# Irish-77/adapting-2D-ViTs-for-3D-point-cloud-understanding

Measured on NVIDIA B200. Metric: tokenized clouds/sec (FPS+kNN+embed), higher is better.
Workload: dtype bf16

## Files before the change

### adapting-2d-vits-for-3d-point-cloud-understanding_b200/csrc/embed_fused.cu

```cuda
#include <vector>

#include "tc_common.cuh"

namespace p3tok {

constexpr int FU_CH_WARPS = 8, FU_OUT_WARPS = 8;
constexpr int FU_THREADS = (3 + FU_CH_WARPS + FU_OUT_WARPS) * 32;
constexpr int FU_CHUNK = 128;
constexpr int FU_CH_BYTES = 2 * 16384;
constexpr int FU_RA_BOX = 64 * 128;
constexpr int FU_MAX_RA = 32, FU_MAX_RB = 16;
constexpr int FU_SMEM = 227 * 1024;
constexpr int FU_L1_WSTRIDE = 76;
constexpr int FU_L1_STAGE = 128 * 16 + 4 * 16;
constexpr int FU_L1_BYTES = 2 * FU_L1_STAGE;

struct FusedParams {
  int M, K0, N1, N2;
  int num_pairs;
  int ra_slots, rb_slots, rb_box;
  int nch;
  int nacc;
  int nq, nq_rows;
  int xtile;
  int a_reuse;
  const float* bias_a;
  const float* gbias;
  int rows_per_group;
  const float* bias_b;
  int store_out;
  float* out_max;
  __nv_bfloat16* out_max_bf16;
  int max_relu;
  unsigned long long* trace;
  const float4* l1_rel;
  const float4* l1_ctr;
  const float* l1_w;
  int l1_relu;
};
__device__ __forceinline__ void fu_trace(const FusedParams& p, int it, int j, int slot, long long v) {
  if (p.trace && blockIdx.x == 0 && it < 4 && j < 16) p.trace[((size_t)it * 16 + j) * 16 + slot] = (unsigned long long)v;
}

__global__ void __launch_bounds__(FU_THREADS, 1)
tc_fused_kernel(const __grid_constant__ CUtensorMap tmA, const __grid_constant__ CUtensorMap tmWa,
                const __grid_constant__ CUtensorMap tmWb, const __grid_constant__ CUtensorMap tmC, const FusedParams p) {
  extern __shared__ uint8_t smem_raw[];
  uint8_t* smem = reinterpret_cast<uint8_t*>((reinterpret_cast<uintptr_t>(smem_raw) + 1023) & ~(uintptr_t)1023);
  const int KB0 = p.K0 / 64, NC = p.N1 / FU_CHUNK, NQ = p.nq;
  uint8_t* sA0 = smem;
  uint8_t* sCH = sA0 + KB0 * 16384;
  uint8_t* sRA = sCH + p.nch * FU_CH_BYTES;
  uint8_t* sRB = sRA + p.ra_slots * FU_RA_BOX;
  uint8_t* sST = sRB + p.rb_slots * p.rb_box;
  float* sba = reinterpret_cast<float*>(sST + (p.store_out ? FU_OUT_WARPS * 4096 : 0));
  float* sbb = sba + p.N1;
  float* sgb = sbb + p.N2;
  const bool L1 = p.l1_rel != nullptr;
  uint8_t* sl1 = reinterpret_cast<uint8_t*>((reinterpret_cast<uintptr_t>(sgb + FU_CH_WARPS * 64) + 15) & ~(uintptr_t)15);
  uint64_t* bars = reinterpret_cast<uint64_t*>((reinterpret_cast<uintptr_t>(sl1 + (L1 ? 2 * FU_L1_STAGE : 0)) + 7) & ~(uintptr_t)7);
  uint64_t* a0_full = bars;
  uint64_t* a0_empty = bars + 1;
  uint64_t* acc3_full = bars + 2;
  uint64_t* acc3_empty = bars + 3;
  uint64_t* acc2_full = bars + 4;
  uint64_t* acc2_empty = bars + 6;
  uint64_t* ch_full = bars + 8;
  uint64_t* ch_empty = bars + 10;
  uint64_t* ra_full = bars + 12;
  uint64_t* ra_empty = bars + 44;
  uint64_t* rb_full = bars + 76;
  uint64_t* rb_empty = bars + 92;
  uint64_t* l1_full = bars + 108;
  uint64_t* l1_empty = bars + 110;
  uint32_t* tmem_slot = reinterpret_cast<uint32_t*>(bars + 112);

  const int warp = __shfl_sync(0xffffffffu, (int)(threadIdx.x >> 5), 0);
  const int lane = threadIdx.x & 31;
  const int rank = (int)cluster_ctarank();
  const int pair_id = blockIdx.x >> 1, pair_stride = gridDim.x >> 1;

  if (threadIdx.x == 0) {
    asm volatile("prefetch.tensormap [%0];" ::"l"(reinterpret_cast<uint64_t>(&tmA)) : "memory");
    asm volatile("prefetch.tensormap [%0];" ::"l"(reinterpret_cast<uint64_t>(&tmWa)) : "memory");
    asm volatile("prefetch.tensormap [%0];" ::"l"(reinterpret_cast<uint64_t>(&tmWb)) : "memory");
    mbar_init(a0_full, L1 ? 2 * FU_CH_WARPS : 1);
    mbar_init(a0_empty, 1);
    for (int b = 0; b < 2; ++b) { mbar_init(&l1_full[b], 1); mbar_init(&l1_empty[b], FU_CH_WARPS); }
    mbar_init(acc3_full, 1);
    mbar_init(acc3_empty, 2 * FU_OUT_WARPS);
    for (int b = 0; b < 2; ++b) {
      mbar_init(&acc2_full[b], 1);
      mbar_init(&acc2_empty[b], 2 * FU_CH_WARPS);
      mbar_init(&ch_full[b], 2 * FU_CH_WARPS);
      mbar_init(&ch_empty[b], 1);
    }
    for (int s = 0; s < FU_MAX_RA; ++s) { mbar_init(&ra_full[s], 1); mbar_init(&ra_empty[s], 1); }
    for (int s = 0; s < FU_MAX_RB; ++s) { mbar_init(&rb_full[s], 1); mbar_init(&rb_empty[s], 1); }
    asm volatile("fence.mbarrier_init.release.cluster;" ::: "memory");
  }
  for (int i = threadIdx.x; i < p.N1; i += FU_THREADS) sba[i] = p.bias_a ? p.bias_a[i] : 0.f;
  int bb_nonzero = 0;
  for (int i = threadIdx.x; i < p.N2; i += FU_THREADS) {
    const float b = p.bias_b ? p.bias_b[i] : 0.f;
    sbb[i] = b;
    bb_nonzero |= (b != 0.f);
  }
  if (warp == 1) {
    asm volatile("tcgen05.alloc.cta_group::2.sync.aligned.shared::cta.b32 [%0], %1;" ::"r"(smem_u32(tmem_slot)), "r"(512));
    asm volatile("tcgen05.relinquish_alloc_permit.cta_group::2.sync.aligned;" ::);
  }
  tc_fence_before();
  const bool has_bb = __syncthreads_or(bb_nonzero) != 0;
  cluster_sync_all();
  tc_fence_after();
  const uint32_t tmem_base = *tmem_slot;
  const int nq_rows = p.nq_rows;
  const uint32_t acc_col0 = 512u - (uint32_t)p.nacc * FU_CHUNK;

  if (warp == 0) {
    const bool issuer = elect_one();
    int rs = 0;
    uint32_t rph = 0;
    int it = 0;
    auto l1_load = [&](int t, int tp_t) {
      const int sb = t & 1;
      mbar_wait(&l1_empty[sb], ((uint32_t)(t >> 1) & 1) ^ 1);
      if (issuer) {
        const int64_t mt_t = 2 * (int64_t)tp_t + rank;
        uint8_t* dst = sl1 + sb * FU_L1_STAGE;
        mbar_expect_tx(&l1_full[sb], (uint32_t)FU_L1_STAGE);
        asm volatile("cp.async.bulk.shared::cluster.global.mbarrier::complete_tx::bytes [%0], [%1], %2, [%3];" ::"r"(smem_u32(dst)),
                     "l"(reinterpret_cast<uint64_t>(p.l1_rel + mt_t * TC_BM)), "r"(128 * 16), "r"(smem_u32(&l1_full[sb]))
                     : "memory");
        asm volatile("cp.async.bulk.shared::cluster.global.mbarrier::complete_tx::bytes [%0], [%1], %2, [%3];" ::"r"(smem_u32(dst + 128 * 16)),
                     "l"(reinterpret_cast<uint64_t>(p.l1_ctr + mt_t * (TC_BM / 32))), "r"(4 * 16), "r"(smem_u32(&l1_full[sb]))
                     : "memory");
      }
      __syncwarp();
    };
    if (L1 && pair_id < p.num_pairs) l1_load(0, pair_id);
    for (int tp = pair_id; tp < p.num_pairs; tp += pair_stride, ++it) {
      const int mt = 2 * tp + rank;
      if (L1) {
        if (tp + pair_stride < p.num_pairs) l1_load(it + 1, tp + pair_stride);
      } else {
        mbar_wait(a0_empty, (uint32_t)(it & 1) ^ 1);
        if (issuer) {
          if (rank == 0) mbar_expect_tx(a0_full, 2u * (uint32_t)KB0 * 16384u);
          for (int kb = 0; kb < KB0; ++kb) tma_load_2d_pair(sA0 + kb * 16384, &tmA, a0_full, kb * 64, mt * TC_BM);
        }
      }
      __syncwarp();
      for (int j = 0; j < NC; ++j) {
        for (int kb = 0; kb < KB0; ++kb) {
          mbar_wait(&ra_empty[rs], rph ^ 1);
          if (issuer) {
            if (rank == 0) mbar_expect_tx(&ra_full[rs], 2u * FU_RA_BOX);
            tma_load_2d_pair(sRA + rs * FU_RA_BOX, &tmWa, &ra_full[rs], kb * 64, j * FU_CHUNK + rank * (FU_CHUNK / 2));
          }
          __syncwarp();
          if (++rs == p.ra_slots) { rs = 0; rph ^= 1; }
        }
      }
    }
  } else if (warp == 2 + FU_CH_WARPS + FU_OUT_WARPS) {
    const bool issuer = elect_one();
    int rs = 0;
    uint32_t rph = 0;
    for (int tp = pair_id; tp < p.num_pairs; tp += pair_stride) {
      for (int j = 0; j < NC; ++j) {
        for (int kq = 0; kq < 2 * NQ; ++kq) {
          const int kb2 = kq / NQ, qd = kq - kb2 * NQ;
          mbar_wait(&rb_empty[rs], rph ^ 1);
          if (issuer) {
            if (rank == 0) mbar_expect_tx(&rb_full[rs], 2u * (uint32_t)p.rb_box);
            tma_load_2d_pair(sRB + rs * p.rb_box, &tmWb, &rb_full[rs], j * FU_CHUNK + kb2 * 64, qd * nq_rows + rank * (nq_rows / 2));
          }
          __syncwarp();
          if (++rs == p.rb_slots) { rs = 0; rph ^= 1; }
        }
      }
    }
  } else if (warp == 1) {
    if (rank == 0) {
      const bool issuer = elect_one();
      const uint64_t dconst = umma_desc_sw128(0);
      const uint32_t idesc_a = (1u << 4) | (1u << 7) | (1u << 10) | ((uint32_t)(FU_CHUNK >> 3) << 17) | ((uint32_t)((2 * TC_BM) >> 4) << 24);
      const uint32_t idesc_b = (1u << 4) | (1u << 7) | (1u << 10) | ((uint32_t)(nq_rows >> 3) << 17) | ((uint32_t)((2 * TC_BM) >> 4) << 24);
      const uint32_t a0_base = smem_u32(sA0) >> 4, ch_base = smem_u32(sCH) >> 4;
      const uint32_t ra_base = smem_u32(sRA) >> 4, rb_base = smem_u32(sRB) >> 4;
      int ras = 0, rbs = 0;
      uint32_t raph = 0, rbph = 0;
      uint32_t gc = 0;
      uint32_t gcb = 0;
      int it = 0;
      auto issue_A = [&](bool last_of_tile) {
        const uint32_t b = p.nacc == 2 ? (gc & 1) : 0u;
        const uint32_t use = p.nacc == 2 ? (gc >> 1) : gc;
        mbar_wait(&acc2_empty[b], (use & 1) ^ 1);
        tc_fence_after();
        const uint32_t d = tmem_base + acc_col0 + b * FU_CHUNK;
        for (int kb = 0; kb < KB0; ++kb) {
          mbar_wait(&ra_full[ras], raph);
          tc_fence_after();
          if (issuer) {
            const uint64_t ad = dconst | (uint64_t)(a0_base + kb * (16384 >> 4));
            const uint64_t bd = dconst | (uint64_t)(ra_base + ras * (FU_RA_BOX >> 4));
#pragma unroll
            for (int k = 0; k < 4; ++k) tc_mma_pair(d, ad + 2 * k, bd + 2 * k, idesc_a, (uint32_t)((kb | k) != 0));
            tc_commit_pair(&ra_empty[ras]);
          }
          __syncwarp();
          if (++ras == p.ra_slots) { ras = 0; raph ^= 1; }
        }
        if (issuer) {
          tc_commit_pair(&acc2_full[b]);
          if (last_of_tile) tc_commit_pair(a0_empty);
        }
        __syncwarp();
        ++gc;
      };
      auto first_A = [&](int tile_it) {
        if (issuer) fu_trace(p, tile_it, 0, 4, clock64());
        mbar_wait(a0_full, (uint32_t)(tile_it & 1));
        if (issuer) fu_trace(p, tile_it, 0, 5, clock64());
        tc_fence_after();
        issue_A(NC == 1);
        if (issuer) fu_trace(p, tile_it, 0, 6, clock64());
      };
      if (p.xtile && pair_id < p.num_pairs) first_A(0);
      for (int tp = pair_id; tp < p.num_pairs; tp += pair_stride, ++it) {
        if (!p.xtile) first_A(it);
        for (int j = 0; j < NC; ++j) {
          if (j + 1 < NC) issue_A(j + 1 == NC - 1);
          else if (p.xtile && tp + pair_stride < p.num_pairs) first_A(it + 1);
          const uint32_t b = p.nch == 2 ? (gcb & 1) : 0u;
          const uint32_t cuse = p.nch == 2 ? (gcb >> 1) : gcb;
          if (issuer) fu_trace(p, it, j, 0, clock64());
          mbar_wait(&ch_full[b], cuse & 1);
          if (issuer) fu_trace(p, it, j, 1, clock64());
          if (j == 0) mbar_wait(acc3_empty, (uint32_t)(it & 1) ^ 1);
          tc_fence_after();
          if (NQ == 2 && p.a_reuse) {
            for (int kb2 = 0; kb2 < 2; ++kb2) {
              const int s0 = rbs;
              const uint32_t ph0 = rbph;
              if (++rbs == p.rb_slots) { rbs = 0; rbph ^= 1; }
              const int s1 = rbs;
              const uint32_t ph1 = rbph;
              if (++rbs == p.rb_slots) { rbs = 0; rbph ^= 1; }
              mbar_wait(&rb_full[s0], ph0);
              if (issuer && kb2 == 0) fu_trace(p, it, j, 2, clock64());
              mbar_wait(&rb_full[s1], ph1);
              if (issuer && kb2 == 1) fu_trace(p, it, j, 3, clock64());
              tc_fence_after();
              if (issuer) {
                const uint64_t ad = dconst | (uint64_t)(ch_base + b * (FU_CH_BYTES >> 4) + kb2 * (16384 >> 4));
                const uint64_t bd0 = dconst | (uint64_t)(rb_base + s0 * (p.rb_box >> 4));
                const uint64_t bd1 = dconst | (uint64_t)(rb_base + s1 * (p.rb_box >> 4));
#pragma unroll
                for (int k = 0; k < 4; ++k) {
                  const uint32_t acc = (uint32_t)((j | kb2 | k) != 0);
                  tc_mma_pair_a<1>(tmem_base, ad + 2 * k, bd0 + 2 * k, idesc_b, acc);
                  tc_mma_pair_a<0>(tmem_base + (uint32_t)nq_rows, ad + 2 * k, bd1 + 2 * k, idesc_b, acc);
                }
                tc_commit_pair(&rb_empty[s0]);
                tc_commit_pair(&rb_empty[s1]);
              }
              __syncwarp();
            }
          } else
          for (int kq = 0; kq < 2 * NQ; ++kq) {
            const int kb2 = kq / NQ, qd = kq - kb2 * NQ;
            mbar_wait(&rb_full[rbs], rbph);
            if (issuer && kq == 0) fu_trace(p, it, j, 2, clock64());
            if (issuer && kq == 2 * NQ - 1) fu_trace(p, it, j, 3, clock64());
            tc_fence_after();
            if (issuer) {
              const uint64_t ad = dconst | (uint64_t)(ch_base + b * (FU_CH_BYTES >> 4) + kb2 * (16384 >> 4));
              const uint64_t bd = dconst | (uint64_t)(rb_base + rbs * (p.rb_box >> 4));
              const uint32_t d = tmem_base + (uint32_t)(qd * nq_rows);
#pragma unroll
              for (int k = 0; k < 4; ++k) tc_mma_pair(d, ad + 2 * k, bd + 2 * k, idesc_b, (uint32_t)((j | kb2 | k) != 0));
              tc_commit_pair(&rb_empty[rbs]);
            }
            __syncwarp();
            if (++rbs == p.rb_slots) { rbs = 0; rbph ^= 1; }
          }
          if (issuer) {
            fu_trace(p, it, j, 7, clock64());
            tc_commit_pair(&ch_empty[b]);
            if (j == NC - 1) tc_commit_pair(acc3_full);
          }
          __syncwarp();
          ++gcb;
        }
      }
    }
  } else if (warp < 2 + FU_CH_WARPS) {
    const int ew = warp - 2;
    const int q = warp & 3, h = ew >> 2;
    const uint32_t lane_field = (uint32_t)(q * 32) << 16;
    const int trow = q * 32 + lane;
    float* my_sgb = sgb + ew * 64;
    uint32_t gc = 0;
    int itc = 0;
    const bool tr = (warp == 2 && lane == 0);
    for (int tp = pair_id; tp < p.num_pairs; tp += pair_stride, ++itc) {
      const int row0 = (2 * tp + rank) * TC_BM + q * 32;
      const float* gb_row = (p.gbias && row0 < p.M) ? p.gbias + (size_t)(row0 / p.rows_per_group) * p.N1 : nullptr;
      for (int j = 0; j < NC; ++j, ++gc) {
        const uint32_t ba = p.nacc == 2 ? (gc & 1) : 0u, use = p.nacc == 2 ? (gc >> 1) : gc;
        const uint32_t bc = p.nch == 2 ? (gc & 1) : 0u, cuse = p.nch == 2 ? (gc >> 1) : gc;
        const int c0 = j * FU_CHUNK + h * 64;
        float2 gpre = make_float2(0.f, 0.f);
        if (gb_row) gpre = __ldg(reinterpret_cast<const float2*>(gb_row + c0) + lane);
        if (tr) fu_trace(p, itc, j, 8, clock64());
        mbar_wait(&acc2_full[ba], use & 1);
        if (tr) fu_trace(p, itc, j, 9, clock64());
        tc_fence_after();
        const uint32_t taddr = tmem_base + lane_field + acc_col0 + ba * FU_CHUNK + h * 64;
        float v[32];
        uint32_t pk[32];
        tc_ld32_issue(taddr, v);
        if (gb_row) {
          *reinterpret_cast<float2*>(my_sgb + 2 * lane) = gpre;
          __syncwarp();
        }
#pragma unroll
        for (int half = 0; half < 2; ++half) {
          tc_ld_wait();
          if (half == 1) {
            tc_fence_before();
            __syncwarp();
            if (lane == 0) mbar_arrive_cta(&acc2_empty[ba], 0);
          }
          const uint32_t sb = smem_u32(sba + c0 + 32 * half), sg = smem_u32(my_sgb + 32 * half);
// ... 59 lines not shown
        for (int c = 0; c < 4; ++c) {
#pragma unroll
          for (int j = 0; j < 8; j += 2) fma2(base[j], base[j + 1], wc[c * 8 + j], wc[c * 8 + j + 1], cv[c], cv[c], base[j], base[j + 1]);
        }
      }
      const float4* relp = reinterpret_cast<const float4*>(sl1 + sb * FU_L1_STAGE) + ew * 16;
      const uint32_t dst0 = smem_u32(sA0) + (uint32_t)(lane >> 3) * 16384u;
#pragma unroll
      for (int r4 = 0; r4 < 16; r4 += 4) {
        uint32_t pk[4][4];
#pragma unroll
        for (int rr = 0; rr < 4; ++rr) {
          const float4 xv = relp[r4 + rr];
          const float xr[4] = {xv.x, xv.y, xv.z, xv.w};
          float a[8];
#pragma unroll
          for (int j = 0; j < 8; ++j) a[j] = base[j];
#pragma unroll
          for (int c = 0; c < 4; ++c) {
#pragma unroll
            for (int j = 0; j < 8; j += 2) fma2(a[j], a[j + 1], wr[c * 8 + j], wr[c * 8 + j + 1], xr[c], xr[c], a[j], a[j + 1]);
          }
#pragma unroll
          for (int j = 0; j < 4; ++j) pk[rr][j] = p.l1_relu ? pack_bf16x2_relu(a[2 * j], a[2 * j + 1]) : pack_bf16x2(a[2 * j], a[2 * j + 1]);
        }
        if (r4 == 0) mbar_wait(a0_empty, (uint32_t)(t & 1) ^ 1);
#pragma unroll
        for (int rr = 0; rr < 4; ++rr) {
          const uint32_t trow_ = (uint32_t)(ew * 16 + r4 + rr);
          const uint32_t dst = dst0 + trow_ * 128u + ((((uint32_t)lane & 7u) ^ (trow_ & 7u)) << 4);
          asm volatile("st.shared.v4.b32 [%0], {%1, %2, %3, %4};" ::"r"(dst), "r"(pk[rr][0]), "r"(pk[rr][1]), "r"(pk[rr][2]), "r"(pk[rr][3]) : "memory");
        }
      }
      asm volatile("fence.proxy.async.shared::cta;" ::: "memory");
      __syncwarp();
      if (lane == 0) {
        mbar_arrive(&l1_empty[sb]);
        mbar_arrive_cta(a0_full, 0);
      }
    };
    if (L1 && pair_id < p.num_pairs) produce_a0(0);
    int it = 0;
    for (int tp = pair_id; tp < p.num_pairs; tp += pair_stride, ++it) {
      if (L1 && tp + pair_stride < p.num_pairs) produce_a0(it + 1);
      const int row0 = (2 * tp + rank) * TC_BM + q * 32;
      const int row = row0 + lane;
      const bool row_ok = row < p.M;
      const int nvalid = p.M - row0 >= 32 ? 32 : (p.M - row0 > 0 ? p.M - row0 : 0);
      const bool tr = (warp == 2 + FU_CH_WARPS && lane == 0);
      if (tr) fu_trace(p, it, 0, 12, clock64());
      mbar_wait(acc3_full, (uint32_t)(it & 1));
      if (tr) fu_trace(p, it, 0, 13, clock64());
      tc_fence_after();
      bool released = false;
      if (!p.store_out) {
        for (int gi = h; gi < ngroups; gi += 2) {
          const int n0 = gi * 64;
          const bool last = gi + 2 >= ngroups;
          float a0[16], b0[16], a1[16], b1[16];
          const uint32_t t0 = tmem_base + lane_field + (uint32_t)n0;
          tc_ld16x256_x4_issue(t0, a0);
          tc_ld16x256_x4_issue(t0 + (16u << 16), b0);
          tc_ld16x256_x4_issue(t0 + 32u, a1);
          tc_ld16x256_x4_issue(t0 + 32u + (16u << 16), b1);
          tc_ld_wait();
          if (last) {
            tc_fence_before();
            __syncwarp();
            if (lane == 0) mbar_arrive_cta(acc3_empty, 0);
            if (tr) fu_trace(p, it, 0, 14, clock64());
            released = true;
          }
          float m0 = rows_max_frag(a0, b0, lane, nvalid) + sbb[n0 + fcol];
          float m1 = rows_max_frag(a1, b1, lane, nvalid) + sbb[n0 + 32 + fcol];
          if (p.max_relu) { m0 = fmaxf(m0, 0.f); m1 = fmaxf(m1, 0.f); }
          if (row0 < p.M) {
            const size_t o = (size_t)(row0 >> 5) * p.N2 + n0 + fcol;
            if (p.out_max) { p.out_max[o] = m0; p.out_max[o + 32] = m1; }
            if (p.out_max_bf16) { p.out_max_bf16[o] = __float2bfloat16_rn(m0); p.out_max_bf16[o + 32] = __float2bfloat16_rn(m1); }
          }
        }
      } else {
        for (int gi = h; gi < ngroups; gi += 2) {
          const int n0 = gi * 64;
          const bool last = gi + 2 >= ngroups;
#pragma unroll
          for (int half = 0; half < 2; ++half) {
            float v[32];
            tc_ld32_issue(tmem_base + lane_field + (uint32_t)(n0 + half * 32), v);
            tc_ld_wait();
            if (last && half == 1) {
              tc_fence_before();
              __syncwarp();
              if (lane == 0) mbar_arrive_cta(acc3_empty, 0);
              if (tr) fu_trace(p, it, 0, 14, clock64());
              released = true;
            }
            if (has_bb) {
#pragma unroll
              for (int i = 0; i < 8; ++i) {
                const float4 b4 = *reinterpret_cast<const float4*>(sbb + n0 + half * 32 + 4 * i);
                v[4 * i] += b4.x; v[4 * i + 1] += b4.y; v[4 * i + 2] += b4.z; v[4 * i + 3] += b4.w;
              }
            }
            if (half == 0) {
              if (lane == 0) asm volatile("cp.async.bulk.wait_group.read 0;" ::: "memory");
              __syncwarp();
            }
            const uint32_t rbase = smem_u32(stg) + lane * 128;
#pragma unroll
            for (int pc = 0; pc < 4; ++pc) {
              const uint32_t a = rbase + (((uint32_t)(pc + 4 * half) ^ (lane & 7)) << 4);
              asm volatile("st.shared.v4.b32 [%0], {%1, %2, %3, %4};" ::"r"(a), "r"(pack_bf16x2(v[pc * 8], v[pc * 8 + 1])),
                           "r"(pack_bf16x2(v[pc * 8 + 2], v[pc * 8 + 3])), "r"(pack_bf16x2(v[pc * 8 + 4], v[pc * 8 + 5])),
                           "r"(pack_bf16x2(v[pc * 8 + 6], v[pc * 8 + 7]))
                           : "memory");
            }
            if (p.out_max) {
              if (!row_ok) {
#pragma unroll
                for (int i = 0; i < 32; ++i) v[i] = -3.0e38f;
              }
              float m = warp_rows_max(v, lane);
              if (p.max_relu) m = fmaxf(m, 0.f);
              if (row0 < p.M) p.out_max[(size_t)(row0 >> 5) * p.N2 + n0 + half * 32 + lane] = m;
            }
          }
          asm volatile("fence.proxy.async.shared::cta;" ::: "memory");
          __syncwarp();
          if (lane == 0 && row0 < p.M) {
            asm volatile("cp.async.bulk.tensor.2d.global.shared::cta.bulk_group [%0, {%2, %3}], [%1];" ::"l"(
                             reinterpret_cast<uint64_t>(&tmC)),
                         "r"(smem_u32(stg)), "r"(n0), "r"(row0)
                         : "memory");
            asm volatile("cp.async.bulk.commit_group;" ::: "memory");
          }
          if (p.out_max_bf16 && row0 < p.M) {
            uint32_t m = box_rows_max_bf16x2(smem_u32(stg), lane, nvalid);
            if (p.max_relu) asm("max.bf16x2 %0, %0, %1;" : "+r"(m) : "r"(0u));
            *reinterpret_cast<uint32_t*>(p.out_max_bf16 + (size_t)(row0 >> 5) * p.N2 + n0 + 2 * lane) = m;
          }
          __syncwarp();
        }
      }
      if (tr) fu_trace(p, it, 0, 15, clock64());
      if (!released) {
        tc_fence_before();
        __syncwarp();
        if (lane == 0) mbar_arrive_cta(acc3_empty, 0);
      }
    }
    if (lane == 0) asm volatile("cp.async.bulk.wait_group 0;" ::: "memory");
  }
  tc_fence_before();
  __syncthreads();
  cluster_sync_all();
  if (warp == 1) {
    tc_fence_after();
    asm volatile("tcgen05.dealloc.cta_group::2.sync.aligned.b32 %0, %1;" ::"r"(tmem_base), "r"(512));
  }
}

static bool fused_rings_n(int K0, int N1, int N2, bool store_out, int nch, bool l1, int& ra_slots, int& rb_slots, int& rb_box) {
  const int nq = N2 > 256 ? 2 : 1;
  rb_box = (N2 / nq / 2) * 128;
  const int fixed = (K0 / 64) * 16384 + nch * FU_CH_BYTES + (store_out ? FU_OUT_WARPS * 4096 : 0) +
                    (N1 + N2 + FU_CH_WARPS * 64) * 4 + (l1 ? FU_L1_BYTES + 16 : 0) + 116 * 8 + 64 + 1024;
  const int left = FU_SMEM - fixed;
  if (left < 2 * FU_RA_BOX + 2 * rb_box) return false;
  const int chunk_a = (K0 / 64) * FU_RA_BOX, chunk_b = 2 * nq * rb_box;
  ra_slots = (int)((int64_t)left * chunk_a / (chunk_a + chunk_b)) / FU_RA_BOX;
  if (ra_slots < 2) ra_slots = 2;
  if (ra_slots > FU_MAX_RA) ra_slots = FU_MAX_RA;
  rb_slots = (left - ra_slots * FU_RA_BOX) / rb_box;
  if (rb_slots > FU_MAX_RB) rb_slots = FU_MAX_RB;
  return rb_slots >= 2;
}

static bool fused_rings(int K0, int N1, int N2, bool store_out, bool l1, int& nch, int& ra_slots, int& rb_slots, int& rb_box) {
  nch = 2;
  if (fused_rings_n(K0, N1, N2, store_out, 2, l1, ra_slots, rb_slots, rb_box) && ra_slots >= 4 && rb_slots >= 3) return true;
  nch = 1;
  return fused_rings_n(K0, N1, N2, store_out, 1, l1, ra_slots, rb_slots, rb_box);
}

bool tc_fused_supported(int K0, int N1, int N2, int64_t rows_per_group, bool has_gbias) {
  if (K0 % 64 || N1 % FU_CHUNK || N2 % 64) return false;
  if (K0 < 64 || K0 > 384 || N2 < 64 || N2 > 384 || N1 < FU_CHUNK || N1 > 2048) return false;
  if (N2 > 256 && (N2 / 2) % 16) return false;
  if (has_gbias && (rows_per_group % 32 != 0)) return false;
  int nch, ra, rb, box;
  return fused_rings(K0, N1, N2, !has_gbias, false, nch, ra, rb, box);
}

__global__ void fused_l1_pack_kernel(const __nv_bfloat16* __restrict__ W, const float* __restrict__ bias, int C, float* __restrict__ out) {
  const int lane = blockIdx.x, i = threadIdx.x;
  float v = 0.f;
  if (i < 64) {
    const int half = i >> 5, c = (i & 31) >> 3, j = i & 7;
    if (c < C) v = __bfloat162float(W[(size_t)(8 * lane + j) * (2 * C) + half * C + c]);
  } else if (i < 72) {
    v = bias ? bias[8 * lane + (i - 64)] : 0.f;
  }
  out[lane * FU_L1_WSTRIDE + i] = v;
}
bool tc_fused_l1_supported(int N1, int N2) {
  if (!tc_fused_supported(256, N1, N2, 32, false)) return false;
  int nch, ra, rb, box;
  return fused_rings(256, N1, N2, true, true, nch, ra, rb, box);
}
int64_t fused_l1_pack_bytes() { return 32 * FU_L1_WSTRIDE * 4; }
int fused_l1_pack(const __nv_bfloat16* W, const float* bias, int C, float* packed, cudaStream_t s) {
  P3_REQUIRE(C == 3 || C == 4, P3TOK_ERR_UNSUPPORTED, "fused_l1_pack: C must be 3 or 4");
  fused_l1_pack_kernel<<<32, FU_L1_WSTRIDE, 0, s>>>(W, bias, C, packed);
  P3_LAUNCH_CHECK("fused_l1_pack_kernel");
  return P3TOK_OK;
}

int tc_fused(const __nv_bfloat16* A0, int64_t M, int K0, const __nv_bfloat16* Wa, int N1, const float* bias_a,
             const float* gbias, int rows_per_group, const __nv_bfloat16* Wb, int N2, const float* bias_b,
             __nv_bfloat16* out_bf16, float* out_max, __nv_bfloat16* out_max_bf16, int max_relu, cudaStream_t s,
             const FusedL1* l1) {
  P3_REQUIRE(tc_fused_supported(K0, N1, N2, rows_per_group, gbias != nullptr), P3TOK_ERR_UNSUPPORTED,
             "tc_fused: unsupported shape K0=%d N1=%d N2=%d", K0, N1, N2);
  P3_REQUIRE(!l1 || (K0 == 256 && l1->rel && l1->ctr && l1->w), P3TOK_ERR_UNSUPPORTED, "tc_fused: the in-kernel first layer needs K0 == 256");
  P3_REQUIRE(M < (1ll << 31) - 512, P3TOK_ERR_UNSUPPORTED, "tc_fused: too many rows");
  if (M == 0) return P3TOK_OK;
  FusedParams p;
  p.M = (int)M; p.K0 = K0; p.N1 = N1; p.N2 = N2;
  const int num_m_tiles = (int)((M + TC_BM - 1) / TC_BM);
  p.num_pairs = (num_m_tiles + 1) / 2;
  p.bias_a = bias_a; p.gbias = gbias; p.rows_per_group = rows_per_group > 0 ? rows_per_group : 32; p.bias_b = bias_b;
  p.store_out = out_bf16 != nullptr; p.out_max = out_max; p.out_max_bf16 = out_max_bf16; p.max_relu = max_relu;
  p.nacc = N2 <= 256 ? 2 : 1;
  p.nq = N2 > 256 ? 2 : 1;
  p.nq_rows = N2 / p.nq;
  static int areuse_on = -1;
  if (areuse_on < 0) { const char* e = getenv("P3TOK_FUSED_AREUSE"); areuse_on = e ? atoi(e) : 1; }
  p.a_reuse = areuse_on && p.nq == 2;
  static int xtile_on = -1;
  if (xtile_on < 0) { const char* e = getenv("P3TOK_FUSED_XTILE"); xtile_on = e ? atoi(e) : 0; }
  p.xtile = xtile_on;
  p.rb_box = (p.nq_rows / 2) * 128;
  P3_REQUIRE(fused_rings(K0, N1, N2, p.store_out != 0, l1 != nullptr, p.nch, p.ra_slots, p.rb_slots, p.rb_box), P3TOK_ERR_UNSUPPORTED,
             "tc_fused: shapes do not fit shared memory");
  p.l1_rel = l1 ? l1->rel : nullptr; p.l1_ctr = l1 ? l1->ctr : nullptr; p.l1_w = l1 ? l1->w : nullptr; p.l1_relu = l1 ? l1->relu : 0;
  CUtensorMap ta, twa, twb, tc;
  int rc = make_map(&twa, Wa, N1, K0, FU_CHUNK / 2);
  if (rc) return rc;
  if (l1) {
    ta = twa;
  } else {
    rc = make_map(&ta, A0, M, K0, TC_BM);
    if (rc) return rc;
  }
  rc = make_map(&twb, Wb, N2, N1, p.nq_rows / 2);
  if (rc) return rc;
  if (out_bf16) {
    rc = make_map(&tc, out_bf16, M, N2, 32);
    if (rc) return rc;
  } else {
    tc = twa;
  }
  static thread_local bool configured[32] = {false};
  int dev = 0;
  P3_CUDA(cudaGetDevice(&dev));
  if (dev < 32 && !configured[dev]) {
    P3_CUDA(cudaFuncSetAttribute(tc_fused_kernel, cudaFuncAttributeMaxDynamicSharedMemorySize, FU_SMEM));
    configured[dev] = true;
  }
  static int trace_on = -1;
  if (trace_on < 0) trace_on = getenv("P3TOK_TC_TRACE") ? 1 : 0;
  p.trace = nullptr;
  const size_t tw = 4 * 16 * 16;
  if (trace_on) {
    P3_CUDA(cudaMalloc(&p.trace, tw * 8));
    P3_CUDA(cudaMemsetAsync(p.trace, 0, tw * 8, s));
  }
  const int max_pairs = num_sms() / 2;
  const int pairs = p.num_pairs < max_pairs ? p.num_pairs : max_pairs;
  cudaLaunchConfig_t cfg = {};
  cfg.gridDim = dim3((unsigned)(pairs * 2));
  cfg.blockDim = dim3(FU_THREADS);
  cfg.dynamicSmemBytes = FU_SMEM;
  cfg.stream = s;
  cudaLaunchAttribute attr[1];
  attr[0].id = cudaLaunchAttributeClusterDimension;
  attr[0].val.clusterDim.x = 2;
  attr[0].val.clusterDim.y = 1;
  attr[0].val.clusterDim.z = 1;
  cfg.attrs = attr;
  cfg.numAttrs = 1;
  P3_CUDA(cudaLaunchKernelEx(&cfg, tc_fused_kernel, ta, twa, twb, tc, p));
  count_launch();
  if (trace_on) {
    std::vector<unsigned long long> h(tw);
    P3_CUDA(cudaStreamSynchronize(s));
    P3_CUDA(cudaMemcpy(h.data(), p.trace, tw * 8, cudaMemcpyDeviceToHost));
    P3_CUDA(cudaFree(p.trace));
    fprintf(stderr, "[fu_trace] M=%d K0=%d N1=%d N2=%d ra=%d rb=%d nch=%d nacc=%d\n", p.M, p.K0, p.N1, p.N2, p.ra_slots, p.rb_slots, p.nch, p.nacc);
    const unsigned long long t0 = h[4];
    auto rel = [&](unsigned long long v) { return v ? (long long)(v - t0) : -1ll; };
    for (int it = 1; it < 3; ++it) {
      const unsigned long long* q = &h[(size_t)it * 16 * 16];
      fprintf(stderr, "[fu_trace] tile%d mma: start=%lld a0_ok=%lld A0_issued=%lld | out-epi: wait=%lld acc3_ok=%lld released=%lld end=%lld\n", it,
              rel(q[4]), rel(q[5]), rel(q[6]), rel(q[12]), rel(q[13]), rel(q[14]), rel(q[15]));
      for (int j = 0; j < 16 && q[j * 16 + 7]; ++j)
        fprintf(stderr, "[fu_trace]   chunk%-2d mma: Anext=%lld ch_ok=%lld wb0=%lld wb3=%lld B=%lld | ch-epi: wait=%lld acc2_ok=%lld conv=%lld pub=%lld\n",
                j, rel(q[j * 16 + 0]), rel(q[j * 16 + 1]), rel(q[j * 16 + 2]), rel(q[j * 16 + 3]), rel(q[j * 16 + 7]),
                rel(q[j * 16 + 8]), rel(q[j * 16 + 9]), rel(q[j * 16 + 10]), rel(q[j * 16 + 11]));
    }
  }
  return P3TOK_OK;
}

}
```

### adapting-2d-vits-for-3d-point-cloud-understanding_b200/csrc/tc_common.cuh

```cuda
#pragma once
#include <cuda.h>
#include <cuda_bf16.h>
#include <stdlib.h>

#include "embed.cuh"

namespace p3tok {

constexpr int TC_BM = 128, TC_BK = 64;

__device__ __forceinline__ uint32_t smem_u32(const void* p) { return (uint32_t)__cvta_generic_to_shared(p); }

__device__ __forceinline__ void mbar_init(uint64_t* bar, uint32_t count) {
  asm volatile("mbarrier.init.shared::cta.b64 [%0], %1;" ::"r"(smem_u32(bar)), "r"(count));
}
__device__ __forceinline__ void mbar_expect_tx(uint64_t* bar, uint32_t bytes) {
  asm volatile("mbarrier.arrive.expect_tx.shared::cta.b64 _, [%0], %1;" ::"r"(smem_u32(bar)), "r"(bytes) : "memory");
}
__device__ __forceinline__ void mbar_arrive(uint64_t* bar) {
  asm volatile("mbarrier.arrive.shared::cta.b64 _, [%0];" ::"r"(smem_u32(bar)) : "memory");
}
__device__ __forceinline__ bool mbar_try_wait(uint64_t* bar, uint32_t parity) {
  uint32_t ok;
  asm volatile(
// ... 9 lines not shown
}
__device__ __forceinline__ void mbar_wait(uint64_t* bar, uint32_t parity) {
  if (mbar_try_wait(bar, parity)) return;
  const long long t0 = clock64();
  while (!mbar_try_wait(bar, parity)) {
    if (clock64() - t0 > 4000000000ll) {
      printf("p3tok: mbarrier wait timed out (block %d thread %d parity %u)\n", (int)blockIdx.x, (int)threadIdx.x, parity);
      __trap();
    }
  }
}
__device__ __forceinline__ void tma_load_2d(void* dst, const CUtensorMap* map, uint64_t* bar, int c0, int c1) {
  asm volatile(
      "cp.async.bulk.tensor.2d.shared::cluster.global.mbarrier::complete_tx::bytes [%0], [%1, {%3, %4}], [%2];" ::"r"(
          smem_u32(dst)),
      "l"(reinterpret_cast<uint64_t>(map)), "r"(smem_u32(bar)), "r"(c0), "r"(c1)
      : "memory");
}
__device__ __forceinline__ void tma_load_2d_mc(void* dst, const CUtensorMap* map, uint64_t* bar, int c0, int c1, uint16_t mask) {
  asm volatile(
      "cp.async.bulk.tensor.2d.shared::cluster.global.mbarrier::complete_tx::bytes.multicast::cluster [%0], [%1, {%3, %4}], [%2], %5;" ::"r"(
          smem_u32(dst)),
      "l"(reinterpret_cast<uint64_t>(map)), "r"(smem_u32(bar)), "r"(c0), "r"(c1), "h"(mask)
      : "memory");
}
__device__ __forceinline__ void tma_prefetch_2d(const CUtensorMap* map, int c0, int c1) {
  asm volatile("cp.async.bulk.prefetch.tensor.2d.L2.global [%0, {%1, %2}];" ::"l"(reinterpret_cast<uint64_t>(map)), "r"(c0), "r"(c1)
               : "memory");
}
__device__ __forceinline__ void tc_commit_mc(uint64_t* bar, uint16_t mask) {
  asm volatile("tcgen05.commit.cta_group::1.mbarrier::arrive::one.shared::cluster.multicast::cluster.b64 [%0], %1;" ::"r"(
                   smem_u32(bar)),
               "h"(mask)
               : "memory");
}
constexpr uint32_t PEER_BIT_MASK = 0xFEFFFFFFu;
__device__ __forceinline__ void tma_load_2d_pair(void* dst, const CUtensorMap* map, uint64_t* leader_bar, int c0, int c1) {
  asm volatile(
      "cp.async.bulk.tensor.2d.cta_group::2.shared::cluster.global.mbarrier::complete_tx::bytes [%0], [%1, {%3, %4}], [%2];" ::"r"(
          smem_u32(dst)),
      "l"(reinterpret_cast<uint64_t>(map)), "r"(smem_u32(leader_bar) & PEER_BIT_MASK), "r"(c0), "r"(c1)
      : "memory");
}
__device__ __forceinline__ void tc_mma_pair(uint32_t tmem_d, uint64_t desc_a, uint64_t desc_b, uint32_t idesc, uint32_t accumulate) {
  asm volatile(
      "{\n\t"
      ".reg .pred p;\n\t"
      "setp.ne.b32 p, %4, 0;\n\t"
      "tcgen05.mma.cta_group::2.kind::f16 [%0], %1, %2, %3, p;\n\t"
      "}" ::"r"(tmem_d),
      "l"(desc_a), "l"(desc_b), "r"(idesc), "r"(accumulate)
      : "memory");
}
template <int KEEP>
__device__ __forceinline__ void tc_mma_pair_a(uint32_t tmem_d, uint64_t desc_a, uint64_t desc_b, uint32_t idesc, uint32_t accumulate) {
  if (KEEP)
    asm volatile(
        "{\n\t"
        ".reg .pred p;\n\t"
        "setp.ne.b32 p, %4, 0;\n\t"
        "tcgen05.mma.cta_group::2.kind::f16.collector::a::fill [%0], %1, %2, %3, p;\n\t"
        "}" ::"r"(tmem_d),
        "l"(desc_a), "l"(desc_b), "r"(idesc), "r"(accumulate)
        : "memory");
  else
    asm volatile(
        "{\n\t"
        ".reg .pred p;\n\t"
        "setp.ne.b32 p, %4, 0;\n\t"
        "tcgen05.mma.cta_group::2.kind::f16.collector::a::lastuse [%0], %1, %2, %3, p;\n\t"
        "}" ::"r"(tmem_d),
        "l"(desc_a), "l"(desc_b), "r"(idesc), "r"(accumulate)
        : "memory");
}
__device__ __forceinline__ void tc_commit_pair(uint64_t* bar) {
  asm volatile("tcgen05.commit.cta_group::2.mbarrier::arrive::one.shared::cluster.multicast::cluster.b64 [%0], %1;" ::"r"(
                   smem_u32(bar)),
               "h"((uint16_t)3)
               : "memory");
}
__device__ __forceinline__ void mbar_arrive_cta(uint64_t* bar, uint32_t cta) {
  asm volatile(
      "{\n\t"
      ".reg .b32 ra;\n\t"
      "mapa.shared::cluster.u32 ra, %0, %1;\n\t"
      "mbarrier.arrive.shared::cluster.b64 _, [ra];\n\t"
      "}" ::"r"(smem_u32(bar)),
      "r"(cta)
      : "memory");
}
__device__ __forceinline__ bool elect_one() {
  uint32_t pred;
  asm volatile(
      "{\n\t"
      ".reg .pred p;\n\t"
      "elect.sync _|p, 0xffffffff;\n\t"
      "selp.u32 %0, 1, 0, p;\n\t"
      "}"
      : "=r"(pred));
  return pred != 0;
}
__device__ __forceinline__ uint32_t cluster_ctarank() {
  uint32_t r;
  asm volatile("mov.u32 %0, %%cluster_ctarank;" : "=r"(r));
  return r;
}
__device__ __forceinline__ void cluster_sync_all() {
  asm volatile("barrier.cluster.arrive.release.aligned;" ::: "memory");
  asm volatile("barrier.cluster.wait.acquire.aligned;" ::: "memory");
}
__device__ __forceinline__ void tc_fence_before() { asm volatile("tcgen05.fence::before_thread_sync;" ::: "memory"); }
__device__ __forceinline__ void tc_fence_after() { asm volatile("tcgen05.fence::after_thread_sync;" ::: "memory"); }
__device__ __forceinline__ void tc_commit(uint64_t* bar) {
  asm volatile("tcgen05.commit.cta_group::1.mbarrier::arrive::one.shared::cluster.b64 [%0];" ::"r"(smem_u32(bar)) : "memory");
// ... 241 lines not shown
```

Measured before the change: 154,300.

## Split second GEMM into thirds with per-third accumulator release and issue order

When N2 is a multiple of 128 and above 256, the second GEMM's N dimension is split into three quarter-boxes instead of two. Each third gets its own acc3_empty barrier. On chunk 0 the B loads and MMAs run third-by-third, so the next tile's accumulation into a third can start as soon as the output epilogue has drained that third, rather than waiting for the whole accumulator. A-collector reuse is extended to fill/use/lastuse across three MMAs, and the unused cross-tile xtile path is removed. The cost is more barriers, smaller B boxes and more MMA instructions per k-step.

```diff
diff --git a/adapting-2d-vits-for-3d-point-cloud-understanding_b200/csrc/embed_fused.cu b/adapting-2d-vits-for-3d-point-cloud-understanding_b200/csrc/embed_fused.cu
--- a/adapting-2d-vits-for-3d-point-cloud-understanding_b200/csrc/embed_fused.cu
+++ b/adapting-2d-vits-for-3d-point-cloud-understanding_b200/csrc/embed_fused.cu
@@ -22,7 +22,6 @@
   int nch;
   int nacc;
   int nq, nq_rows;
-  int xtile;
   int a_reuse;
   const float* bias_a;
   const float* gbias;
@@ -38,8 +37,9 @@
   const float* l1_w;
   int l1_relu;
 };
+constexpr int FU_TRACE_SLOTS = 17;
 __device__ __forceinline__ void fu_trace(const FusedParams& p, int it, int j, int slot, long long v) {
-  if (p.trace && blockIdx.x == 0 && it < 4 && j < 16) p.trace[((size_t)it * 16 + j) * 16 + slot] = (unsigned long long)v;
+  if (p.trace && blockIdx.x == 0 && it < 4 && j < 16) p.trace[((size_t)it * 16 + j) * FU_TRACE_SLOTS + slot] = (unsigned long long)v;
 }
 
 __global__ void __launch_bounds__(FU_THREADS, 1)
@@ -48,6 +48,7 @@
   extern __shared__ uint8_t smem_raw[];
   uint8_t* smem = reinterpret_cast<uint8_t*>((reinterpret_cast<uintptr_t>(smem_raw) + 1023) & ~(uintptr_t)1023);
   const int KB0 = p.K0 / 64, NC = p.N1 / FU_CHUNK, NQ = p.nq;
+  const int NREL = NQ == 3 ? 3 : 1;
   uint8_t* sA0 = smem;
   uint8_t* sCH = sA0 + KB0 * 16384;
   uint8_t* sRA = sCH + p.nch * FU_CH_BYTES;
@@ -63,17 +64,17 @@
   uint64_t* a0_empty = bars + 1;
   uint64_t* acc3_full = bars + 2;
   uint64_t* acc3_empty = bars + 3;
-  uint64_t* acc2_full = bars + 4;
-  uint64_t* acc2_empty = bars + 6;
-  uint64_t* ch_full = bars + 8;
-  uint64_t* ch_empty = bars + 10;
-  uint64_t* ra_full = bars + 12;
-  uint64_t* ra_empty = bars + 44;
-  uint64_t* rb_full = bars + 76;
-  uint64_t* rb_empty = bars + 92;
-  uint64_t* l1_full = bars + 108;
-  uint64_t* l1_empty = bars + 110;
-  uint32_t* tmem_slot = reinterpret_cast<uint32_t*>(bars + 112);
+  uint64_t* acc2_full = bars + 6;
+  uint64_t* acc2_empty = bars + 8;
+  uint64_t* ch_full = bars + 10;
+  uint64_t* ch_empty = bars + 12;
+  uint64_t* ra_full = bars + 14;
+  uint64_t* ra_empty = bars + 46;
+  uint64_t* rb_full = bars + 78;
+  uint64_t* rb_empty = bars + 94;
+  uint64_t* l1_full = bars + 110;
+  uint64_t* l1_empty = bars + 112;
+  uint32_t* tmem_slot = reinterpret_cast<uint32_t*>(bars + 114);
 
   const int warp = __shfl_sync(0xffffffffu, (int)(threadIdx.x >> 5), 0);
   const int lane = threadIdx.x & 31;
@@ -88,7 +89,7 @@
     mbar_init(a0_empty, 1);
     for (int b = 0; b < 2; ++b) { mbar_init(&l1_full[b], 1); mbar_init(&l1_empty[b], FU_CH_WARPS); }
     mbar_init(acc3_full, 1);
-    mbar_init(acc3_empty, 2 * FU_OUT_WARPS);
+    for (int q = 0; q < 3; ++q) mbar_init(&acc3_empty[q], 2 * FU_OUT_WARPS);
     for (int b = 0; b < 2; ++b) {
       mbar_init(&acc2_full[b], 1);
       mbar_init(&acc2_empty[b], 2 * FU_CH_WARPS);
@@ -170,8 +171,9 @@
     uint32_t rph = 0;
     for (int tp = pair_id; tp < p.num_pairs; tp += pair_stride) {
       for (int j = 0; j < NC; ++j) {
+        const bool third_major = NREL > 1 && j == 0;
         for (int kq = 0; kq < 2 * NQ; ++kq) {
-          const int kb2 = kq / NQ, qd = kq - kb2 * NQ;
+          const int kb2 = third_major ? (kq & 1) : kq / NQ, qd = third_major ? (kq >> 1) : kq - kb2 * NQ;
           mbar_wait(&rb_empty[rs], rph ^ 1);
           if (issuer) {
             if (rank == 0) mbar_expect_tx(&rb_full[rs], 2u * (uint32_t)p.rb_box);
@@ -221,58 +223,70 @@
         __syncwarp();
         ++gc;
       };
-      auto first_A = [&](int tile_it) {
-        if (issuer) fu_trace(p, tile_it, 0, 4, clock64());
-        mbar_wait(a0_full, (uint32_t)(tile_it & 1));
-        if (issuer) fu_trace(p, tile_it, 0, 5, clock64());
+      for (int tp = pair_id; tp < p.num_pairs; tp += pair_stride, ++it) {
+        if (issuer) fu_trace(p, it, 0, 4, clock64());
+        mbar_wait(a0_full, (uint32_t)(it & 1));
+        if (issuer) fu_trace(p, it, 0, 5, clock64());
         tc_fence_after();
         issue_A(NC == 1);
-        if (issuer) fu_trace(p, tile_it, 0, 6, clock64());
-      };
-      if (p.xtile && pair_id < p.num_pairs) first_A(0);
-      for (int tp = pair_id; tp < p.num_pairs; tp += pair_stride, ++it) {
-        if (!p.xtile) first_A(it);
+        if (issuer) fu_trace(p, it, 0, 6, clock64());
         for (int j = 0; j < NC; ++j) {
           if (j + 1 < NC) issue_A(j + 1 == NC - 1);
-          else if (p.xtile && tp + pair_stride < p.num_pairs) first_A(it + 1);
           const uint32_t b = p.nch == 2 ? (gcb & 1) : 0u;
           const uint32_t cuse = p.nch == 2 ? (gcb >> 1) : gcb;
           if (issuer) fu_trace(p, it, j, 0, clock64());
           mbar_wait(&ch_full[b], cuse & 1);
           if (issuer) fu_trace(p, it, j, 1, clock64());
-          if (j == 0) mbar_wait(acc3_empty, (uint32_t)(it & 1) ^ 1);
+          const bool third_major = NREL > 1 && j == 0;
+          if (j == 0 && !third_major) mbar_wait(&acc3_empty[0], (uint32_t)(it & 1) ^ 1);
           tc_fence_after();
-          if (NQ == 2 && p.a_reuse) {
+          if (NQ > 1 && p.a_reuse && !third_major) {
             for (int kb2 = 0; kb2 < 2; ++kb2) {
-              const int s0 = rbs;
-              const uint32_t ph0 = rbph;
-              if (++rbs == p.rb_slots) { rbs = 0; rbph ^= 1; }
-              const int s1 = rbs;
-              const uint32_t ph1 = rbph;
-              if (++rbs == p.rb_slots) { rbs = 0; rbph ^= 1; }
-              mbar_wait(&rb_full[s0], ph0);
-              if (issuer && kb2 == 0) fu_trace(p, it, j, 2, clock64());
-              mbar_wait(&rb_full[s1], ph1);
-              if (issuer && kb2 == 1) fu_trace(p, it, j, 3, clock64());
+              int s[3];
+              uint32_t ph[3];
+#pragma unroll
+              for (int q = 0; q < 3; ++q) {
+                if (q < NQ) {
+                  s[q] = rbs;
+                  ph[q] = rbph;
+                  if (++rbs == p.rb_slots) { rbs = 0; rbph ^= 1; }
+                }
+              }
+#pragma unroll
+              for (int q = 0; q < 3; ++q) {
+                if (q < NQ) {
+                  mbar_wait(&rb_full[s[q]], ph[q]);
+                  if (issuer && kb2 == 0 && q == 0) fu_trace(p, it, j, 2, clock64());
+                  if (issuer && kb2 == 1 && q == NQ - 1) fu_trace(p, it, j, 3, clock64());
+                }
+              }
               tc_fence_after();
               if (issuer) {
                 const uint64_t ad = dconst | (uint64_t)(ch_base + b * (FU_CH_BYTES >> 4) + kb2 * (16384 >> 4));
-                const uint64_t bd0 = dconst | (uint64_t)(rb_base + s0 * (p.rb_box >> 4));
-                const uint64_t bd1 = dconst | (uint64_t)(rb_base + s1 * (p.rb_box >> 4));
+                const uint64_t bd0 = dconst | (uint64_t)(rb_base + s[0] * (p.rb_box >> 4));
+                const uint64_t bd1 = dconst | (uint64_t)(rb_base + s[1] * (p.rb_box >> 4));
+                const uint64_t bdl = NQ == 3 ? dconst | (uint64_t)(rb_base + s[2] * (p.rb_box >> 4)) : bd1;
+                const uint32_t dl = tmem_base + (uint32_t)((NQ - 1) * nq_rows);
 #pragma unroll
                 for (int k = 0; k < 4; ++k) {
                   const uint32_t acc = (uint32_t)((j | kb2 | k) != 0);
-                  tc_mma_pair_a<1>(tmem_base, ad + 2 * k, bd0 + 2 * k, idesc_b, acc);
-                  tc_mma_pair_a<0>(tmem_base + (uint32_t)nq_rows, ad + 2 * k, bd1 + 2 * k, idesc_b, acc);
+                  tc_mma_pair_a<A_FILL>(tmem_base, ad + 2 * k, bd0 + 2 * k, idesc_b, acc);
+                  if (NQ == 3) tc_mma_pair_a<A_USE>(tmem_base + (uint32_t)nq_rows, ad + 2 * k, bd1 + 2 * k, idesc_b, acc);
+                  tc_mma_pair_a<A_LASTUSE>(dl, ad + 2 * k, bdl + 2 * k, idesc_b, acc);
                 }
-                tc_commit_pair(&rb_empty[s0]);
-                tc_commit_pair(&rb_empty[s1]);
+#pragma unroll
+                for (int q = 0; q < 3; ++q)
+                  if (q < NQ) tc_commit_pair(&rb_empty[s[q]]);
               }
               __syncwarp();
             }
           } else
           for (int kq = 0; kq < 2 * NQ; ++kq) {
-            const int kb2 = kq / NQ, qd = kq - kb2 * NQ;
+            const int kb2 = third_major ? (kq & 1) : kq / NQ, qd = third_major ? (kq >> 1) : kq - kb2 * NQ;
+            if (third_major && kb2 == 0) {
+              mbar_wait(&acc3_empty[qd], (uint32_t)(it & 1) ^ 1);
+              tc_fence_after();
+            }
             mbar_wait(&rb_full[rbs], rbph);
             if (issuer && kq == 0) fu_trace(p, it, j, 2, clock64());
             if (issuer && kq == 2 * NQ - 1) fu_trace(p, it, j, 3, clock64());
@@ -284,6 +298,7 @@
 #pragma unroll
               for (int k = 0; k < 4; ++k) tc_mma_pair(d, ad + 2 * k, bd + 2 * k, idesc_b, (uint32_t)((j | kb2 | k) != 0));
               tc_commit_pair(&rb_empty[rbs]);
+              if (third_major && kb2 == 1) fu_trace(p, it, qd, 16, clock64());
             }
             __syncwarp();
             if (++rbs == p.rb_slots) { rbs = 0; rbph ^= 1; }
@@ -449,11 +464,16 @@
       mbar_wait(acc3_full, (uint32_t)(it & 1));
       if (tr) fu_trace(p, it, 0, 13, clock64());
       tc_fence_after();
-      bool released = false;
+      auto release = [&](int rq) {
+        tc_fence_before();
+        __syncwarp();
+        if (lane == 0) mbar_arrive_cta(&acc3_empty[rq], 0);
+        if (tr) fu_trace(p, it, rq, 14, clock64());
+      };
       if (!p.store_out) {
         for (int gi = h; gi < ngroups; gi += 2) {
           const int n0 = gi * 64;
-          const bool last = gi + 2 >= ngroups;
+          const bool rel = NREL > 1 || gi + 2 >= ngroups;
           float a0[16], b0[16], a1[16], b1[16];
           const uint32_t t0 = tmem_base + lane_field + (uint32_t)n0;
           tc_ld16x256_x4_issue(t0, a0);
@@ -461,13 +481,7 @@
           tc_ld16x256_x4_issue(t0 + 32u, a1);
           tc_ld16x256_x4_issue(t0 + 32u + (16u << 16), b1);
           tc_ld_wait();
-          if (last) {
-            tc_fence_before();
-            __syncwarp();
-            if (lane == 0) mbar_arrive_cta(acc3_empty, 0);
-            if (tr) fu_trace(p, it, 0, 14, clock64());
-            released = true;
-          }
+          if (rel) release(NREL > 1 ? gi >> 1 : 0);
           float m0 = rows_max_frag(a0, b0, lane, nvalid) + sbb[n0 + fcol];
           float m1 = rows_max_frag(a1, b1, lane, nvalid) + sbb[n0 + 32 + fcol];
           if (p.max_relu) { m0 = fmaxf(m0, 0.f); m1 = fmaxf(m1, 0.f); }
@@ -480,19 +494,13 @@
       } else {
         for (int gi = h; gi < ngroups; gi += 2) {
           const int n0 = gi * 64;
-          const bool last = gi + 2 >= ngroups;
+          const bool rel = NREL > 1 || gi + 2 >= ngroups;
 #pragma unroll
           for (int half = 0; half < 2; ++half) {
             float v[32];
             tc_ld32_issue(tmem_base + lane_field + (uint32_t)(n0 + half * 32), v);
             tc_ld_wait();
-            if (last && half == 1) {
-              tc_fence_before();
-              __syncwarp();
-              if (lane == 0) mbar_arrive_cta(acc3_empty, 0);
-              if (tr) fu_trace(p, it, 0, 14, clock64());
-              released = true;
-            }
+            if (rel && half == 1) release(NREL > 1 ? gi >> 1 : 0);
             if (has_bb) {
 #pragma unroll
               for (int i = 0; i < 8; ++i) {
@@ -541,11 +549,7 @@
         }
       }
       if (tr) fu_trace(p, it, 0, 15, clock64());
-      if (!released) {
-        tc_fence_before();
-        __syncwarp();
-        if (lane == 0) mbar_arrive_cta(acc3_empty, 0);
-      }
+      if (h >= ngroups) release(0);
     }
     if (lane == 0) asm volatile("cp.async.bulk.wait_group 0;" ::: "memory");
   }
@@ -558,8 +562,10 @@
   }
 }
 
+static int fused_nq(int N2) { return N2 <= 256 ? 1 : (N2 % 128 == 0 ? 3 : 2); }
+
 static bool fused_rings_n(int K0, int N1, int N2, bool store_out, int nch, bool l1, int& ra_slots, int& rb_slots, int& rb_box) {
-  const int nq = N2 > 256 ? 2 : 1;
+  const int nq = fused_nq(N2);
   rb_box = (N2 / nq / 2) * 128;
   const int fixed = (K0 / 64) * 16384 + nch * FU_CH_BYTES + (store_out ? FU_OUT_WARPS * 4096 : 0) +
                     (N1 + N2 + FU_CH_WARPS * 64) * 4 + (l1 ? FU_L1_BYTES + 16 : 0) + 116 * 8 + 64 + 1024;
@@ -584,7 +590,7 @@
 bool tc_fused_supported(int K0, int N1, int N2, int64_t rows_per_group, bool has_gbias) {
   if (K0 % 64 || N1 % FU_CHUNK || N2 % 64) return false;
   if (K0 < 64 || K0 > 384 || N2 < 64 || N2 > 384 || N1 < FU_CHUNK || N1 > 2048) return false;
-  if (N2 > 256 && (N2 / 2) % 16) return false;
+  if (fused_nq(N2) == 2 && (N2 / 2) % 16) return false;
   if (has_gbias && (rows_per_group % 32 != 0)) return false;
   int nch, ra, rb, box;
   return fused_rings(K0, N1, N2, !has_gbias, false, nch, ra, rb, box);
@@ -630,14 +636,11 @@
   p.bias_a = bias_a; p.gbias = gbias; p.rows_per_group = rows_per_group > 0 ? rows_per_group : 32; p.bias_b = bias_b;
   p.store_out = out_bf16 != nullptr; p.out_max = out_max; p.out_max_bf16 = out_max_bf16; p.max_relu = max_relu;
   p.nacc = N2 <= 256 ? 2 : 1;
-  p.nq = N2 > 256 ? 2 : 1;
+  p.nq = fused_nq(N2);
   p.nq_rows = N2 / p.nq;
   static int areuse_on = -1;
   if (areuse_on < 0) { const char* e = getenv("P3TOK_FUSED_AREUSE"); areuse_on = e ? atoi(e) : 1; }
-  p.a_reuse = areuse_on && p.nq == 2;
-  static int xtile_on = -1;
-  if (xtile_on < 0) { const char* e = getenv("P3TOK_FUSED_XTILE"); xtile_on = e ? atoi(e) : 0; }
-  p.xtile = xtile_on;
+  p.a_reuse = areuse_on && p.nq > 1;
   p.rb_box = (p.nq_rows / 2) * 128;
   P3_REQUIRE(fused_rings(K0, N1, N2, p.store_out != 0, l1 != nullptr, p.nch, p.ra_slots, p.rb_slots, p.rb_box), P3TOK_ERR_UNSUPPORTED,
              "tc_fused: shapes do not fit shared memory");
@@ -669,7 +672,7 @@
   static int trace_on = -1;
   if (trace_on < 0) trace_on = getenv("P3TOK_TC_TRACE") ? 1 : 0;
   p.trace = nullptr;
-  const size_t tw = 4 * 16 * 16;
+  const size_t tw = 4 * 16 * FU_TRACE_SLOTS;
   if (trace_on) {
     P3_CUDA(cudaMalloc(&p.trace, tw * 8));
     P3_CUDA(cudaMemsetAsync(p.trace, 0, tw * 8, s));
@@ -695,17 +698,22 @@
     P3_CUDA(cudaStreamSynchronize(s));
     P3_CUDA(cudaMemcpy(h.data(), p.trace, tw * 8, cudaMemcpyDeviceToHost));
     P3_CUDA(cudaFree(p.trace));
-    fprintf(stderr, "[fu_trace] M=%d K0=%d N1=%d N2=%d ra=%d rb=%d nch=%d nacc=%d\n", p.M, p.K0, p.N1, p.N2, p.ra_slots, p.rb_slots, p.nch, p.nacc);
+    fprintf(stderr, "[fu_trace] M=%d K0=%d N1=%d N2=%d ra=%d rb=%d rb_box=%d nq=%d nch=%d nacc=%d\n", p.M, p.K0, p.N1, p.N2, p.ra_slots,
+            p.rb_slots, p.rb_box, p.nq, p.nch, p.nacc);
+    const int S = FU_TRACE_SLOTS, nrel = p.nq == 3 ? 3 : 1;
     const unsigned long long t0 = h[4];
     auto rel = [&](unsigned long long v) { return v ? (long long)(v - t0) : -1ll; };
     for (int it = 1; it < 3; ++it) {
-      const unsigned long long* q = &h[(size_t)it * 16 * 16];
+      const unsigned long long* q = &h[(size_t)it * 16 * S];
       fprintf(stderr, "[fu_trace] tile%d mma: start=%lld a0_ok=%lld A0_issued=%lld | out-epi: wait=%lld acc3_ok=%lld released=%lld end=%lld\n", it,
-              rel(q[4]), rel(q[5]), rel(q[6]), rel(q[12]), rel(q[13]), rel(q[14]), rel(q[15]));
-      for (int j = 0; j < 16 && q[j * 16 + 7]; ++j)
+              rel(q[4]), rel(q[5]), rel(q[6]), rel(q[12]), rel(q[13]), rel(q[(nrel - 1) * S + 14]), rel(q[15]));
+      if (nrel == 3)
+        fprintf(stderr, "[fu_trace]   thirds: chunk0 issued=%lld/%lld/%lld | out-epi released=%lld/%lld/%lld\n", rel(q[16]), rel(q[S + 16]),
+                rel(q[2 * S + 16]), rel(q[14]), rel(q[S + 14]), rel(q[2 * S + 14]));
+      for (int j = 0; j < 16 && q[j * S + 7]; ++j)
         fprintf(stderr, "[fu_trace]   chunk%-2d mma: Anext=%lld ch_ok=%lld wb0=%lld wb3=%lld B=%lld | ch-epi: wait=%lld acc2_ok=%lld conv=%lld pub=%lld\n",
-                j, rel(q[j * 16 + 0]), rel(q[j * 16 + 1]), rel(q[j * 16 + 2]), rel(q[j * 16 + 3]), rel(q[j * 16 + 7]),
-                rel(q[j * 16 + 8]), rel(q[j * 16 + 9]), rel(q[j * 16 + 10]), rel(q[j * 16 + 11]));
+                j, rel(q[j * S + 0]), rel(q[j * S + 1]), rel(q[j * S + 2]), rel(q[j * S + 3]), rel(q[j * S + 7]),
+                rel(q[j * S + 8]), rel(q[j * S + 9]), rel(q[j * S + 10]), rel(q[j * S + 11]));
     }
   }
   return P3TOK_OK;
diff --git a/adapting-2d-vits-for-3d-point-cloud-understanding_b200/csrc/tc_common.cuh b/adapting-2d-vits-for-3d-point-cloud-understanding_b200/csrc/tc_common.cuh
--- a/adapting-2d-vits-for-3d-point-cloud-understanding_b200/csrc/tc_common.cuh
+++ b/adapting-2d-vits-for-3d-point-cloud-understanding_b200/csrc/tc_common.cuh
@@ -85,14 +85,24 @@
       "l"(desc_a), "l"(desc_b), "r"(idesc), "r"(accumulate)
       : "memory");
 }
-template <int KEEP>
+enum ACollector { A_FILL, A_USE, A_LASTUSE };
+template <ACollector C>
 __device__ __forceinline__ void tc_mma_pair_a(uint32_t tmem_d, uint64_t desc_a, uint64_t desc_b, uint32_t idesc, uint32_t accumulate) {
-  if (KEEP)
+  if (C == A_FILL)
     asm volatile(
         "{\n\t"
         ".reg .pred p;\n\t"
         "setp.ne.b32 p, %4, 0;\n\t"
         "tcgen05.mma.cta_group::2.kind::f16.collector::a::fill [%0], %1, %2, %3, p;\n\t"
+        "}" ::"r"(tmem_d),
+        "l"(desc_a), "l"(desc_b), "r"(idesc), "r"(accumulate)
+        : "memory");
+  else if (C == A_USE)
+    asm volatile(
+        "{\n\t"
+        ".reg .pred p;\n\t"
+        "setp.ne.b32 p, %4, 0;\n\t"
+        "tcgen05.mma.cta_group::2.kind::f16.collector::a::use [%0], %1, %2, %3, p;\n\t"
         "}" ::"r"(tmem_d),
         "l"(desc_a), "l"(desc_b), "r"(idesc), "r"(accumulate)
         : "memory");
```

Result: slower. 139,900, median of 6 (-9.3%).
